# zhiqiangdon/pose-adv-aug

Measured on AMD Instinct MI355X. Metric: images/sec, 2-stack HG 256x256 bs=24 per GPU, full training step, higher is better.
Workload: dtype bf16; 1 GPU; BASELINE configs[1]: 2-stack hourglass chan 256, bs=24/GPU, 256x256 MPII-shape synthetic frames (720x1280 uint8 resident in HBM), on-device HumanAug warp, heat-map MSE, RMSprop, PCKh; global_batch=24, parallelism=dp1, ranks_seen=1, devices_seen=1

## Files before the change

### include/poseadv.h

```cpp
#ifndef POSEADV_H
#define POSEADV_H
#include <stddef.h>
#include <stdint.h>
#ifdef __cplusplus
extern "C" {
#endif

const char* pa_last_error(void);
int pa_version(void);
int pa_dtype(void);
float pa_grad_scale(void);


int pa_gaussian_heatmap(const double* pts, float* out, int B, int J, int H, int W, void* stream);

int pa_weighted_l2(const float* pred, const float* gt, const float* weight, size_t n, float* loss, void* stream);
int pa_weighted_l2_grad(const float* pred, const float* gt, const float* weight, size_t n, const float* gout_dev,
                        float* dpred, void* stream);

int pa_get_preds(const float* maps, int B, int J, int H, int W, float* preds, float* maxval, void* stream);

int pa_final_preds(const float* maps, const float* center, const float* scale, const float* rot,
                   int B, int J, int H, int W, float* out, float* scratch_preds, void* stream);

// ... 160 lines not shown
int pa_hg_set_dropout_masks(pa_net* net, const float* masks);

int pa_hg_accuracy(pa_net* net, int stack, const int32_t* idxs, int nidx, float* acc, float* scratch);

int pa_hg_pckh(pa_net* net, int stack, const float* center, const float* scale, const float* rot, const float* gt_pts,
               const float* norm, const int32_t* idxs, int nidx, float* acc, float* person, float* scratch);

int pa_net_meters_async(pa_net* net, int on);

#define PA_PROF_CLASSES 12
int pa_net_profile_begin(pa_net* net);
int pa_net_profile_report(pa_net* net, double* out_host, int cap_classes, int* n_classes);
int pa_net_profile_classes(const pa_net* net, int32_t* out_host, int cap);
int pa_net_set_fin_prologue(pa_net* net, int max_rows);
int pa_net_set_pool_route(pa_net* net, int on);
int pa_net_design_bytes(const pa_net* net, double* out_host);
int pa_copy_probe(void* dst, const void* src, size_t bytes, void* stream);
int pa_copy_probe_form(void* dst, const void* src, size_t bytes, int form, void* stream);
int pa_conv2d_time(int mode, int variant, int B, int Cin, int Cout, int H, int W, int k, int iters, void* ws, float* ms_out, void* stream);
int pa_conv_plan_describe(int B, int H, int W, int Cin, int Cout, int taps, int in_mode, int add1_mode, int add2_mode, int ep_mode,
                          int ep2_mode, int fin_rows, int flags, int cus, int* out, int cap);
int pa_conv_launch_log(int* out, int cap);

int pa_net_set_multi_stream(pa_net* net, int on);

int pa_hg_debug_tensor(pa_net* net, const char* which, int grad, float* out, int* shape4);

int pa_asn_debug_tensor(pa_net* net, const char* which, int grad, float* out, int* shape4);

#ifdef __cplusplus
// ... 4 lines not shown
```

### pose_adv_aug_amd/_lib.py

```python
import ctypes as C
import os

import torch

_HERE = os.path.dirname(os.path.abspath(__file__))
DTYPE = os.environ.get('POSEADV_DTYPE', 'bf16').lower()
if DTYPE not in ('bf16', 'fp16'):
    raise ValueError('POSEADV_DTYPE must be bf16 or fp16')
LIB_PATH = os.path.join(_HERE, 'libposeadv_hip.so' if DTYPE == 'bf16' else 'libposeadv_hip_fp16.so')


def set_dtype(name):
    global DTYPE, LIB_PATH
    name = name.lower()
    if name not in ('bf16', 'fp16'):
        raise ValueError('dtype must be bf16 or fp16')
    if _lib is not None and name != DTYPE:
        raise PoseAdvError('the %s library is already loaded in this process' % DTYPE)
    DTYPE = name
    LIB_PATH = os.path.join(_HERE, 'libposeadv_hip.so' if name == 'bf16' else 'libposeadv_hip_fp16.so')


def act_dtype():
    return torch.bfloat16 if DTYPE == 'bf16' else torch.float16
# ... 120 lines not shown
    'pa_hg_forward_half': (_i, [_vp, _vp, _vp, _i]),
    'pa_asn_forward': (_i, [_vp, _vp, _i, _vp, _vp]),
    'pa_asn_probs': (_vp, [_vp]),
    'pa_asn_backward': (_i, [_vp, _vp, _vp, _vp, _vp]),
    'pa_asn_set_log_eps': (_i, [_vp, _f]),
    'pa_hg_pckh': (_i, [_vp, _i, _vp, _vp, _vp, _vp, _vp, _vp, _i, _vp, _vp, _vp]),
    'pa_net_meters_async': (_i, [_vp, _i]),
    'pa_net_profile_begin': (_i, [_vp]),
    'pa_net_profile_report': (_i, [_vp, C.POINTER(C.c_double), _i, C.POINTER(_i)]),
    'pa_net_design_bytes': (_i, [_vp, C.POINTER(C.c_double)]),
    'pa_copy_probe': (_i, [_vp, _vp, _sz, _vp]),
    'pa_copy_probe_form': (_i, [_vp, _vp, _sz, _i, _vp]),
    'pa_params_csr': (_i, [_vp, _i, _vp, _vp]),
    'pa_net_set_fin_prologue': (_i, [_vp, _i]),
    'pa_net_set_pool_route': (_i, [_vp, _i]),
    'pa_wgrad_group_workspace_bytes': (_sz, [_vp, _i]),
    'pa_wgrad_group': (_i, [_vp, _i, _i, _vp, _vp]),
    'pa_conv2d_time': (_i, [_i] * 9 + [_vp, C.POINTER(C.c_float), _vp]),
    'pa_conv_plan_describe': (_i, [_i] * 14 + [C.POINTER(_i), _i]),
    'pa_conv_launch_log': (_i, [C.POINTER(_i), _i]),
    'pa_net_profile_classes': (_i, [_vp, C.POINTER(C.c_int32), _i]),
    'pa_net_set_multi_stream': (_i, [_vp, _i]),
    'pa_hg_debug_tensor': (_i, [_vp, C.c_char_p, _i, _vp, C.POINTER(_i)]),
    'pa_asn_debug_tensor': (_i, [_vp, C.c_char_p, _i, _vp, C.POINTER(_i)]),
}

EXPORTS = sorted(_PROTOS)


def lib():
# ... 49 lines not shown
```

### pose_adv_aug_amd/csrc/api.hip

```cpp
#include "../../include/poseadv.h"
#include "net.h"
#include "warp_bwd.h"
#include <stdio.h>
#include <string.h>
#include <new>
#include <string>

static thread_local char g_err[1024] = "";
void pa_set_error(const char* what, hipError_t e, const char* file, int line) {
    snprintf(g_err, sizeof g_err, "%s:%d: %s -> %s", file, line, what, hipGetErrorString(e));
}
void pa_set_error_msg(const char* msg) { snprintf(g_err, sizeof g_err, "%s", msg); }

struct pa_net { Net n; };
#define ST(s) reinterpret_cast<hipStream_t>(s)
#define TRY(x) do { int _r = (x); if (_r) { if (!g_err[0]) pa_set_error("kernel launch", (hipError_t)_r, __FILE__, __LINE__); return _r; } } while (0)

extern "C" {

const char* pa_last_error(void) { return g_err; }
float pa_grad_scale(void) { return PA_GRAD_SCALE; }
int pa_dtype(void) { return PA_DTYPE_ID; }
int pa_version(void) { return 1; }

// ... 810 lines not shown
    for (int c = 0; c < PA_PROF_NCLS && c < cap_classes; ++c)
        for (int j = 0; j < 4; ++j) out[c * 4 + j] = full[c * 4 + j];
    if (n_classes) *n_classes = PA_PROF_NCLS;
    return 0;
}
int pa_net_set_fin_prologue(pa_net* net, int max_rows) {
    net->n.fin_rows_max = max_rows < 0 ? 0 : (max_rows > PA_FIN_SMALL_ROWS ? PA_FIN_SMALL_ROWS : max_rows);
    net->n.release_graph();
    return 0;
}
int pa_net_set_pool_route(pa_net* net, int on) {
    net->n.pool_route = on ? 3 : 0;
    net->n.release_graph();
    return 0;
}
int pa_net_design_bytes(const pa_net* net, double* out) { out[0] = net->n.dbytes_rd; out[1] = net->n.dbytes_wr; return 0; }

int pa_net_profile_classes(const pa_net* net, int32_t* out, int cap) {
    const std::vector<int>& q = net->n.prof.last_seq;
    for (int i = 0; i < cap && i < (int)q.size(); ++i) out[i] = q[i];
    return (int)q.size();
}

int pa_net_set_multi_stream(pa_net* net, int on) {
    if (net->n.ensure_streams()) return 1;
    net->n.release_graph();
    net->n.multi_stream = on != 0 && net->n.side != nullptr;
    return 0;
}

// ... 64 lines not shown
                if (out && h.routed[k]) TRY(h.fill_poolgrad(n, k, n.xin[i]));
                head.raw = h.poolgrad[k]; head.B = x.B; head.H = x.H; head.W = x.W; head.C = x.C; a = &head;
            }
        } else {
            int k = r[r.find_first_of("1234")] - '1';
            std::string rest = r.substr(r.find_first_of("1234") + 1);
            if (r.rfind("skip", 0) == 0) a = pick_chain(h.skip[k], rest);
            else if (r.rfind("down", 0) == 0) a = pick_chain(h.down[k], rest);
            else if (r.rfind("up", 0) == 0) a = pick_chain(h.up[k], rest);
            else if (r.rfind("pool", 0) == 0) a = &h.pooled[k];
            else if (r.rfind("merge", 0) == 0) a = &h.merged[k];
        }
    }
    if (bad_block) { pa_set_error_msg("pa_hg_debug_tensor: no such block in the site's chain"); return 1; }
    if (!a) { pa_set_error_msg("pa_hg_debug_tensor: unknown tensor name"); return 1; }
    return debug_copy(n, *a, grad, out, shape4, "pa_hg_debug_tensor", mat);
}


int pa_asn_debug_tensor(pa_net* net, const char* which, int grad, float* out, int* shape4) {
    Net& n = net->n;
    std::string w(which);
    const Act* a = nullptr;
    const bf16* mat = nullptr;
    auto pick = [&](Residual& r, const std::string& rest) -> const Act* {
        if (rest == ".x1") return &r.x1;
        if (rest == ".x2") { mat = r.dz2_valid ? r.dz2 : nullptr; return &r.x2; }
        mat = r.dz3_valid ? r.dz3 : nullptr;
        return &r.x3;
    };
// ... 11 lines not shown
```

### pose_adv_aug_amd/csrc/conv_igemm.hip

```cpp
#include "common.h"
#include "kernels.h"
#include "common.h"
PA_STAMP_DECL(pa_conv1_clk, pa_debug_conv1_clocks)
#define PA_STAMP1(i) PA_STAMP_AT(pa_conv1_clk, a.dbg & 64, i)
#define PA_EPI_STAMP(i) PA_STAMP1(i)
#include "conv_epilogue.h"
#include <string.h>

template <int BM, int BN, int LDMODE, int TAPS, bool STEM = false, bool FIN = false>
__global__ __launch_bounds__(256, FIN ? 2 : 1) void conv_igemm_kernel(PaConvArgs a) {
    constexpr int AI = BM / 32, BI = BN / 32;
    constexpr int MI = BM / 32, NI = BN / 32;
    __shared__ __attribute__((aligned(16))) bf16 lds[(BM + BN) * 64];
    __shared__ float kst[LDMODE == PA_LD_PLAIN ? 4 : 3 * 512 + (FIN ? 2048 : 0)];
    bf16* As = lds;
    bf16* Bs = lds + BM * 64;
    const int tid = threadIdx.x, lane = tid & 63, wave = tid >> 6;
    const int wm = wave & 1, wn = wave >> 1;
    const int M = a.B * a.H * a.W, HW = a.H * a.W;
    const int K = TAPS * a.Cin;
    const int nK = K / 64;
    const int m0 = blockIdx.x * BM, n0 = blockIdx.y * BN;
    const int cc = tid & 7, r = tid >> 3;

// ... 281 lines not shown
}

template <int BM, int BN, int TAPS>
static void launch_ld(const PaConvArgs& a, int variant, dim3 grid, hipStream_t st) {
    if constexpr (BM == 64 && BN == 64) {
        if (variant == PA_CV_BNRELU_FIN) { hipLaunchKernelGGL((conv_igemm_kernel<BM, BN, PA_LD_BNRELU, TAPS, false, true>), grid, dim3(256), 0, st, a); return; }
        if (variant == PA_CV_LIN2_FIN) { hipLaunchKernelGGL((conv_igemm_kernel<BM, BN, PA_LD_LIN2, TAPS, false, true>), grid, dim3(256), 0, st, a); return; }
    }
    switch (variant) {
        case PA_LD_PLAIN: hipLaunchKernelGGL((conv_igemm_kernel<BM, BN, PA_LD_PLAIN, TAPS>), grid, dim3(256), 0, st, a); break;
        case PA_LD_BNRELU: hipLaunchKernelGGL((conv_igemm_kernel<BM, BN, PA_LD_BNRELU, TAPS>), grid, dim3(256), 0, st, a); break;
        default: hipLaunchKernelGGL((conv_igemm_kernel<BM, BN, PA_LD_LIN2, TAPS>), grid, dim3(256), 0, st, a); break;
    }
}

int pa_launch_stem_conv(const PaConvArgs& a, hipStream_t st, int* stat_rows) {
    if (a.Cin != 256 || a.Cout != 64 || a.in.mode != PA_LD_PLAIN) { pa_set_error_msg("pa_launch_stem_conv: bad arguments"); return 1; }
    const int M = a.B * a.H * a.W;
    const int bm = pa_conv_big_m(M) ? 128 : 64, rows = (M + bm - 1) / bm;
    if (stat_rows) *stat_rows = rows; if (a.ep.rows_out) *a.ep.rows_out = rows;
    if (bm == 128) hipLaunchKernelGGL((conv_igemm_kernel<128, 64, PA_LD_PLAIN, 1, true>), dim3(rows, 1), dim3(256), 0, st, a);
    else hipLaunchKernelGGL((conv_igemm_kernel<64, 64, PA_LD_PLAIN, 1, true>), dim3(rows, 1), dim3(256), 0, st, a);
    return (int)hipGetLastError();
}

static int g_log[1024][14], g_nlog = -1;
static void log_launch(const PaConvShape& s) {
    const int r[14] = {s.B, s.H, s.W, s.Cin, s.Cout, s.taps, s.in_mode, s.add1_mode, s.add2_mode, s.ep_mode, s.ep2_mode, s.fin_rows,
                       s.bias | s.out2 << 1 | s.want_dz << 2 | s.in_map << 3 | s.in_q << 4 | s.ep2_affine << 5 | s.add2_map << 6, s.cus};
    int i = 0; while (i < g_nlog && memcmp(g_log[i], r, sizeof r)) ++i;
    if (i == g_nlog && i < 1024) memcpy(g_log[g_nlog++], r, sizeof r);
}
int pa_launch_conv(const PaConvArgs& a0, const PaConvPlan& p, hipStream_t st, int* stat_rows) {
    if (p.path == PA_CVP_REFUSED) { pa_set_error_msg(p.why); return 1; }
    if (g_nlog >= 0) log_launch(pa_conv_shape(a0));
// ... 41 lines not shown
```

### pose_adv_aug_amd/csrc/kernels.h

```cpp
#pragma once
#include "common.h"
#include "bn_fin.h"
#include "launch_plan.h"
#include "wgrad_plan.h"
#include "conv_plan.h"

struct PaConvArgs {
    PaOperand in;
    const bf16* w;
    const float* bias;
    PaOperand add1;
    PaOperand add2;
    PaEpilogue ep;
    bf16* out;
    int B, H, W, Cin, Cout, taps;
    bf16* dz_out;
    PaBnFin fin;
    int low_prio;
    int dbg;
    int xcd;
    PaEpilogue ep2;
    bf16* out2;
};
int pa_conv_cus();
// ... 45 lines not shown
int pa_launch_bn_bwd_finalize(const float* bstats, int rows, const float* scale, const float* mean, const float* invstd,
                              float* kA, float* kB, float* kC, float* dgamma, float* dbeta, int C, float count,
                              hipStream_t st);

int pa_launch_maxpool_fwd(const PaOperand& in, bf16* out, int B, int H, int W, int C, hipStream_t st, unsigned char* map = nullptr, bf16* xmax = nullptr);
bool pa_pool_stats_route_supported(const PaOperand& in, const PaEpilogue& ep, int B, int H, int W, int C);
int pa_launch_maxpool_bwd_stats(const bf16* dout, const bf16* xmax, const PaOperand& in, const PaEpilogue& ep, int B, int H, int W, int C,
                                hipStream_t st, int* stat_rows = nullptr);
int pa_launch_maxpool_bwd(const bf16* dout, const PaOperand& in, const PaOperand& add, const PaEpilogue& ep, bf16* din,
                          int B, int H, int W, int C, hipStream_t st, int* stat_rows = nullptr);
int pa_launch_upadd_fwd(const PaOperand& low, const PaOperand& skip, bf16* out, int B, int H, int W, int C, hipStream_t st);
int pa_launch_upadd_bwd(const bf16* dout, const PaEpilogue& ep_low, bf16* dlow, const PaEpilogue& ep_skip, bf16* dskip,
                        int B, int H, int W, int C, hipStream_t st, int* stat_rows = nullptr, int part = 3);
bool pa_upadd_bwd_splits(const PaEpilogue& ep_low, const PaEpilogue& ep_skip, int B, int H, int W, int C);

int pa_launch_stem_conv(const PaConvArgs& a, hipStream_t st, int* stat_rows = nullptr);
int pa_launch_stem_wgrad(const PaWgradArgs& a, hipStream_t st);
int pa_launch_stem_wgrad_reduce(const float* part, int splits, float* dst, hipStream_t st, float* zero64 = nullptr);

struct PaStemDgradArgs {
    PaOperand g;
    const bf16* wf;
    float* out;
    int B, Hm, Wm, layout;
    float scale;
};
int pa_launch_stem_dgrad(const PaStemDgradArgs& a, hipStream_t st);
int pa_launch_stem_pack(const float* w, bf16* wf, hipStream_t st);

int pa_launch_rmsprop(float* p, const float* g, float* v, size_t n, float lr, float alpha, float eps, float gscale, int* state, hipStream_t st);
struct PaRmspropOpts { float lr, alpha, eps, mom, wd; };
// ... 26 lines not shown
```

### pose_adv_aug_amd/csrc/net.h

```cpp
#pragma once
#include <string>
#include <vector>
#include "common.h"
#include "kernels.h"
#include "pose_ops.h"

struct Arena {
    char* base = nullptr;
    size_t off = 0;
    void* take(size_t bytes) {
        off = (off + 255) & ~(size_t)255;
        void* p = base ? base + off : nullptr;
        off += bytes;
        return p;
    }
    template <typename T> T* get(size_t n) { return reinterpret_cast<T*>(take(n * sizeof(T))); }
};

struct TensorInfo {
    std::string name;
    int shape[4];
    int ndim;
    size_t offset;
    size_t numel;
// ... 8 lines not shown
    float *scale = nullptr, *shift = nullptr, *mean = nullptr, *invstd = nullptr;
    float *kA = nullptr, *kB = nullptr, *kC = nullptr;
    bool fin_pending = false, bfin_pending = false;
};

struct ConvLayer {
    int Cin = 0, Cout = 0, k = 1;
    int pcin = 0, pcout = 0;
    size_t p_w = 0, p_b = 0;
    bf16 *wf = nullptr, *wb = nullptr;
    float *part = nullptr, *dbpart = nullptr;
    int splits = 0;
    int red_index = -1;
    size_t part_floats = 0, db_floats = 0;
    bool has_bn_after = true;
    int taps() const { return k * k; }
};

struct Act {
    bf16* raw = nullptr;
    bf16* grad = nullptr;
    BNLayer* bn = nullptr;
    int B = 0, H = 0, W = 0, C = 0;
    size_t numel() const { return (size_t)B * H * W * C; }
    int M() const { return B * H * W; }
};

struct Net;

enum { PA_PROF_FWD1 = 0, PA_PROF_FWD3, PA_PROF_DGRAD1, PA_PROF_DGRAD3, PA_PROF_WGRAD1, PA_PROF_WGRAD3, PA_PROF_STEM_FWD,
// ... 170 lines not shown
    int finish_grad(const Act& a);
    int finish_grad2(const Act& a, const Act& b);
    int conv_fwd(ConvLayer& c, const PaOperand& in, int B, int H, int W, const PaOperand& add1, const PaOperand& add2,
                 bf16* out, BNLayer* bn_after, BNLayer* pending_in = nullptr, bool defer_after = false);
    int conv_dgrad(ConvLayer& c, const PaOperand& dy, int B, int H, int W, const PaOperand& add1, const PaOperand& add2,
                   const PaEpilogue& ep, bf16* out, bf16* dz_out = nullptr, bool* dz_done = nullptr, BNLayer* pending_in = nullptr,
                   const Act* low = nullptr, bool* low_done = nullptr,
                   const PaEpilogue* pool_in_ep = nullptr);
    int fin_rows_max = pa_tuning().fin_prologue > PA_FIN_SMALL_ROWS ? PA_FIN_SMALL_ROWS : pa_tuning().fin_prologue;
    int pool_route = pa_tuning().pool_route;
    bool maps_on = false;
    unsigned char* stem_map = nullptr; bf16* stem_xmax = nullptr;
    bool stem_map_written = false, stem_routed = false;
    bool stem_route_ok();
    int fill_stem_grad();
    int fin_mask = pa_tuning().fin_mask;
    bool fin_consumer_ok(const ConvLayer& c, int B, int H, int W, bool dgrad) const;
    PaBnFin fin_fwd(const BNLayer& b, int M) const;
    PaBnFin fin_bwd(const BNLayer& b, int M) const;
    int finish_grad_or_defer(const Act& a, bool defer);
    int finish_grad2_or_defer(const Act& a, bool defer_a, const Act& b, bool defer_b);
    bool x3_fin_ok(const Residual& r, const Act& in) const;
    bool x3_fin_ok(const Chain& c, const Act& in) const { return x3_fin_ok(c.tail(), c.tail_in(in)); }
    int conv_wgrad(ConvLayer& c, const PaOperand& dy, const PaOperand& x, int B, int H, int W);

    int prepare_weights();
    int begin_step();
    const bf16* cur_image = nullptr;
    int forward_pose(const float* img_nchw, const bf16* img4_in, const double* pts, bool train, float* loss_out_dev);
    int forward_pose_body(const float* img_nchw, const bf16* img4_in, const double* pts, bool train, float* loss_out_dev);
    int backward_pose();
    int backward_stack(int i);
    int backward_stem();
    hipEvent_t ev_bucket[16], ev_bucket_main = nullptr; bool bucket_events = false;
    int mark_bucket(int stack);
    int reduce_grads();
    int forward_half(const float* img_nchw, const bf16* img4_in, bool train);

    int scale_num = 7, rot_num = 7;
    Residual asn_in[5];
// ... 21 lines not shown
```

### pose_adv_aug_amd/csrc/net.hip

```cpp
#include "net.h"
#include <stdio.h>
#include <string.h>

static int ablate() { return pa_tuning().ablate; }
static int ablate_h() { return pa_tuning().ablate_h; }
#define TRY(x) do { int _r = (x); if (_r) return _r; } while (0)

PaOperand pa_plain(const bf16* p) { PaOperand o; o.p = p; o.q = nullptr; o.k0 = o.k1 = o.k2 = nullptr; o.map = nullptr; o.mode = PA_LD_PLAIN; return o; }
PaOperand pa_none() { PaOperand o; o.p = o.q = nullptr; o.k0 = o.k1 = o.k2 = nullptr; o.map = nullptr; o.mode = PA_LD_NONE; return o; }
static PaEpilogue ep_plain() { PaEpilogue e; memset(&e, 0, sizeof e); e.mode = PA_OUT_PLAIN; return e; }
static int round64(int v) { return (v + 63) / 64 * 64; }

size_t Net::add_param(const std::string& name, std::initializer_list<int> shape) {
    TensorInfo t; t.name = name; t.ndim = (int)shape.size(); t.is_buffer = 0;
    size_t n = 1; int i = 0;
    for (int s : shape) { t.shape[i++] = s; n *= (size_t)s; }
    for (; i < 4; ++i) t.shape[i] = 1;
    n_params = (n_params + 3) & ~(size_t)3;
    t.offset = n_params; t.numel = n;
    n_params += n;
    tensors.push_back(t);
    return t.offset;
}

// ... 185 lines not shown
        lgrad_tmp[i] = a.get<bf16>((size_t)M * chan);
        if (i + 1 < stacks) {
            layout_conv(forth[i], a, M, H4, H4); layout_conv(inc[i], a, M, H4, H4);
            forth_tmp[i] = a.get<bf16>((size_t)M * chan);
        }
        if (i == 0) xin[0] = res3.x3;
        if (i + 1 < stacks) xin[i + 1] = new_act(a, B, H4, H4, chan, nullptr, true);
    }
    a.take(0);
    return a.off;
}

int Net::upload_tables() {
    std::vector<PaPrepJob> pj; std::vector<PaWgradReduceJob> rj; std::vector<PaBnEvalJob> bj;
    prep_max = 0; red_max = 0;
    for (ConvLayer* c : convs) {
        PaPrepJob p; p.w = params + c->p_w; p.wf = c->wf; p.wb = c->wb; p.Cout = c->Cout; p.Cin = c->Cin;
        p.taps = c->k == 7 ? 49 : c->taps(); p.pad_cout = c->pcout; p.pad_cin = c->pcin;
        pj.push_back(p);
        int pe = c->pcout * (c->k == 7 ? 256 : c->taps() * c->pcin);
        if (pe > prep_max) prep_max = pe;
        if (c->k == 7) continue;
        PaWgradReduceJob r; r.part = c->part; r.dst = grads + c->p_w; r.dbpart = c->dbpart; r.dbdst = grads + c->p_b;
        r.Cout = c->pcout; r.Cin = c->pcin; r.taps = c->taps(); r.splits = c->splits; r.real_cout = c->Cout; r.real_cin = c->Cin;
        c->red_index = (int)rj.size();
        rj.push_back(r);
        int re = c->Cout * c->Cin * c->taps() + c->Cout;
        if (re > red_max) red_max = re;
    }
    for (BNLayer* b : bns) {
// ... 120 lines not shown
    f.scale = b.scale; f.shift = b.shift; f.mean = b.mean; f.invstd = b.invstd;
    f.momentum = momentum; f.eps = eps; f.update_running = bn_update;
    return f;
}

PaBnFin Net::fin_bwd(const BNLayer& b, int M) const {
    PaBnFin f; memset(&f, 0, sizeof f);
    f.stats = b.bstats; f.rows = b.bstat_rows; f.bwd = 1; f.count = (float)M;
    f.scale = b.scale; f.mean = b.mean; f.invstd = b.invstd;
    f.kA = b.kA; f.kB = b.kB; f.kC = b.kC; f.dgamma = grads + b.p_gamma; f.dbeta = grads + b.p_beta;
    return f;
}

int Net::conv_fwd(ConvLayer& c, const PaOperand& in, int B_, int H, int W, const PaOperand& add1, const PaOperand& add2,
                  bf16* out, BNLayer* bn_after, BNLayer* pending_in, bool defer_after) {
    PaConvArgs a; memset(&a, 0, sizeof a);
    if (pending_in && pending_in->fin_pending) { a.fin = fin_fwd(*pending_in, B_ * H * W); pending_in->fin_pending = false; }
    a.in = in; a.w = c.wf; a.bias = params + c.p_b; a.add1 = add1; a.add2 = add2; a.out = out; a.low_prio = on_side ? 1 : 0;
    a.B = B_; a.H = H; a.W = W; a.Cin = c.pcin; a.Cout = c.pcout; a.taps = c.k == 7 ? 1 : c.taps();
    a.ep = ep_plain();
    if (bn_after && train_bn) { a.ep.mode = PA_OUT_STATS; a.ep.stats = bn_after->stats; a.ep.rows_out = &bn_after->stat_rows; }
    double wb, wf; conv_work(B_ * H * W, c.k == 7 ? 147 : c.Cin, c.Cout, c.k == 7 ? 1 : c.taps(), false, wb, wf);
    if (c.k == 7) wb = 2.0 * B_ * (4.0 * H * W * 4 + (double)H * W * 64) + 2.0 * 64 * 147;
    if ((ablate() & 128) && H <= ablate_h()) return 0;
    { const double M = (double)B_ * H * W;
      cnt((c.k == 7 ? 2.0 * B_ * 4.0 * H * W * 4 : opb(in, M * a.Cin)) + opb(add1, M * a.Cout) + opb(add2, M * a.Cout) + 2.0 * a.Cout * a.taps * a.Cin, 2.0 * M * a.Cout); }
    ProfEntry* pe = prof.begin(c.k == 7 ? PA_PROF_STEM_FWD : ((long)B_ * H * W < PA_PROF_LOW_M ? PA_PROF_LOW_FWD : (c.k == 3 ? PA_PROF_FWD3 : PA_PROF_FWD1)), wb, wf, st);
    int rc = (c.k == 3 && (ablate() & 8)) ? 0 : ((c.k == 7) ? pa_launch_stem_conv(a, st) : pa_launch_conv(a, st));
    prof.end(pe, st);
    TRY(rc);
    if (bn_after && train_bn && defer_after && bn_after->stat_rows > 0 && bn_after->stat_rows <= fin_rows_max) { bn_after->fin_pending = true; return 0; }
    if (bn_after && train_bn && !(ablate() & 4))
        TRY(pa_launch_bn_finalize(bn_after->stats, bn_after->stat_rows, params + bn_after->p_gamma, params + bn_after->p_beta,
                                  buffers + bn_after->b_rmean, buffers + bn_after->b_rvar, bn_after->scale, bn_after->shift,
                                  bn_after->mean, bn_after->invstd, bn_after->C, (float)(B_ * H * W), momentum, eps, bn_update, st));
    return 0;
}

int Net::conv_dgrad(ConvLayer& c, const PaOperand& dy, int B_, int H, int W, const PaOperand& add1, const PaOperand& add2,
                    const PaEpilogue& ep, bf16* out, bf16* dz_out, bool* dz_done, BNLayer* pending_in, const Act* low, bool* low_done,
                    const PaEpilogue* pool_in_ep) {
    PaConvArgs a; memset(&a, 0, sizeof a);
    if (low_done) *low_done = false;
    if (pending_in && pending_in->bfin_pending) { a.fin = fin_bwd(*pending_in, B_ * H * W); pending_in->bfin_pending = false; }
    a.in = dy; a.w = c.wb; a.bias = nullptr; a.add1 = add1; a.add2 = add2; a.out = out; a.ep = ep; a.low_prio = on_side ? 1 : 0;
    a.B = B_; a.H = H; a.W = W; a.Cin = c.pcout; a.Cout = c.pcin; a.taps = c.taps();
    if (dy.mode == PA_LD_POOL) {
        if (!pool_in_ep || !dz_out) { pa_set_error_msg("conv_dgrad: a pool-routed gradient needs its mask and a dz buffer"); return 1; }
        a.ep2 = *pool_in_ep;
    }
    if (dy.mode == PA_LD_POOL || dy.mode == PA_LD_LIN2) a.dz_out = dz_out;
    if (low && dy.mode != PA_LD_POOL && pa_tuning().upadd_fuse && low->bn && !drop_mask && !(ablate() & 1024)) { a.out2 = low->grad; a.ep2 = final_ep(*low); }
    PaConvPlan p = pa_conv_plan(pa_conv_shape(a));
    if (a.out2 && p.path != PA_CVP_ROW_UP) { a.out2 = nullptr; memset(&a.ep2, 0, sizeof a.ep2); p = pa_conv_plan(pa_conv_shape(a)); }
    const bool up = p.path == PA_CVP_ROW_UP; if (dz_done) *dz_done = p.stores_dz;
    double wb, wf; conv_work(B_ * H * W, c.Cin, c.Cout, c.taps(), false, wb, wf);
// ... 383 lines not shown
        }
        if (k >= 1) TRY(n.finish_grad_or_defer(x, n.x3_fin_ok(down[k - 1], pooled[k - 1])));
        else TRY(n.finish_grad(x));
    }
    return 0;
}

int Net::ensure_streams() {
    if (streams_ready) return 0;
    if (pa_tuning().single_stream) { streams_ready = true; return 0; }
    PA_CHECK(hipStreamCreateWithFlags(&side, hipStreamNonBlocking));
    for (int k = 0; k < 4; ++k) {
        PA_CHECK(hipEventCreateWithFlags(&ev_fork[k], hipEventDisableTiming));
        PA_CHECK(hipEventCreateWithFlags(&ev_join[k], hipEventDisableTiming));
    }
    if (!pa_tuning().no_wstream) {
        PA_CHECK(hipStreamCreateWithFlags(&wstream, hipStreamNonBlocking));
        for (int i = 0; i < 16; ++i) PA_CHECK(hipEventCreateWithFlags(&ev_w[i], hipEventDisableTiming));
        PA_CHECK(hipEventCreateWithFlags(&ev_wdone, hipEventDisableTiming));
    }
    streams_ready = true;
    return 0;
}
void Net::release_streams() {
    release_graph();
    if (bucket_events) { for (int i = 0; i < 16; ++i) (void)hipEventDestroy(ev_bucket[i]); (void)hipEventDestroy(ev_bucket_main); bucket_events = false; }
    if (mstream) { (void)hipStreamSynchronize(mstream); (void)hipStreamDestroy(mstream); (void)hipEventDestroy(ev_mfork); (void)hipEventDestroy(ev_meter); mstream = nullptr; meter_pending = false; }
    if (side) {
        (void)hipStreamSynchronize(side); (void)hipStreamDestroy(side); side = nullptr;
        for (int k = 0; k < 4; ++k) { (void)hipEventDestroy(ev_fork[k]); (void)hipEventDestroy(ev_join[k]); }
    }
    if (wstream) {
        (void)hipStreamSynchronize(wstream); (void)hipStreamDestroy(wstream); wstream = nullptr;
        for (int i = 0; i < 16; ++i) (void)hipEventDestroy(ev_w[i]);
        (void)hipEventDestroy(ev_wdone);
    }
    for (ProfEntry& e : prof.entries) { (void)hipEventDestroy(e.e0); (void)hipEventDestroy(e.e1); }
    prof.entries.clear(); prof.used = 0;
    streams_ready = false;
}
int Net::fork_to(int k) { PA_CHECK(hipEventRecord(ev_fork[k], st)); PA_CHECK(hipStreamWaitEvent(side, ev_fork[k], 0)); return 0; }
int Net::record_join(int k) { PA_CHECK(hipEventRecord(ev_join[k], side)); return 0; }
int Net::wait_join(int k) { PA_CHECK(hipStreamWaitEvent(st, ev_join[k], 0)); return 0; }

int Net::prepare_weights() { return pa_launch_weight_prep(prep_jobs, n_prep, prep_max, st); }

int Net::begin_step() {
    dbytes_rd = dbytes_wr = 0;
    if (!loss_self_clearing) PA_CHECK(hipMemsetAsync(stats_arena, 0, stats_arena_floats * sizeof(float), st));
    return 0;
}

int Net::meter_stream(hipStream_t* out) {
    *out = st;
    if (!meters_async || !multi_stream) return join_meters();
    if (!mstream) {
        PA_CHECK(hipStreamCreateWithFlags(&mstream, hipStreamNonBlocking));
        PA_CHECK(hipEventCreateWithFlags(&ev_mfork, hipEventDisableTiming));
        PA_CHECK(hipEventCreateWithFlags(&ev_meter, hipEventDisableTiming));
    }
// ... 43 lines not shown
    if (!img4_in) TRY(pa_launch_nchw_to_nhwc4(img_nchw, img4, B, res, res, st));
    if (pts && pts != pts_dev) PA_CHECK(hipMemcpyAsync(pts_dev, pts, (size_t)B * classes * 2 * sizeof(double), hipMemcpyDeviceToDevice, st));
    TRY(conv_fwd(stem_conv, pa_plain(image), B, res / 2, res / 2, pa_none(), pa_none(), a0.raw, &stem_bn));
    TRY(res1.fwd(*this, a0));
    maps_on = (pool_route & 1) && train;
    stem_map_written = (pool_route & 2) && train && stem_map && pa_pool_stats_route_supported(op(res1.x3), final_ep(res1.x3), B, res / 2, res / 2, 128);
    TRY(c_maxpool_fwd(*this, op(res1.x3), pool0.raw, B, res / 2, res / 2, 128, st, stem_map_written ? stem_map : nullptr, stem_map_written ? stem_xmax : nullptr));
    TRY(res2.fwd(*this, pool0));
    TRY(res3.fwd(*this, res2.x3));
    const int Hh = res / 4;
    for (int i = 0; i < stacks; ++i) {
        TRY(hg[i].encode(*this, xin[i]));
        TRY(hg[i].decode(*this));
        TRY(post[i].fwd(*this, hg[i].out()));
        TRY(conv_fwd(lin[i], op(post[i].out()), B, Hh, Hh, pa_none(), pa_none(), lin_out[i].raw, &lin_bn[i]));
        TRY(c_head_fwd(*this, op(lin_out[i]), outc[i].wf, params + outc[i].p_b, heat[i], heat64[i], pts ? pts_dev : nullptr,
                               pts ? loss_dev + i : nullptr, B, Hh, Hh, chan, st));
        if (i + 1 < stacks) {
            TRY(conv_fwd(forth[i], op(lin_out[i]), B, Hh, Hh, op(xin[i]), pa_none(), forth_tmp[i], nullptr));
            TRY(conv_fwd(inc[i], pa_plain(heat64[i]), B, Hh, Hh, pa_plain(forth_tmp[i]), pa_none(), xin[i + 1].raw, nullptr));
        }
    }
    if (pts) TRY(pa_launch_loss_out(loss_dev, loss_keep, loss_out_dev, loss_total_out, stacks, st));
    return 0;
}

int Net::backward_stack(int i) {
    const int Hh = res / 4;
    const float gscale = PA_GRAD_SCALE / ((float)B * 16.f * (float)Hh * (float)Hh);
    const bool inner = i + 1 < stacks;
// ... 20 lines not shown
    TRY(finish_grad(lin_out[i]));
    PaOperand gl = gradop(lin_out[i]);
    bool gl_stored = false;
    TRY(conv_dgrad(lin[i], gl, B, Hh, Hh, pa_none(), pa_none(), final_ep(post[i].out()), post[i].out().grad, lgrad_tmp[i], &gl_stored));
    if (gl_stored) gl = pa_plain(lgrad_tmp[i]);
    TRY(conv_wgrad(lin[i], gl, op(post[i].out()), B, Hh, Hh));
    TRY(finish_grad(post[i].out()));
    post[i].head().low_of_in = hg[i].low_fusable(*this, 0) ? &hg[i].up[0].out() : nullptr;
    TRY(post[i].bwd(*this, hg[i].out(), pa_none(), true));
    hg[i].low_done[0] = post[i].head().low_fused;
    TRY(hg[i].bwd(*this, xin[i], inner ? pa_plain(xin[i + 1].grad) : pa_none()));
    return 0;
}

int Net::backward_stem() {
    TRY(res3.bwd(*this, res2.x3, pa_none(), true));
    TRY(finish_grad(res2.x3));
    TRY(res2.bwd(*this, pool0, pa_none(), true));
    stem_routed = stem_route_ok();
    res1.g3_pool_on = stem_routed;
    if (stem_routed) {
        const double e = (double)B * (res / 4) * (res / 4) * 128;
        cnt(4.0 * e, 0.0);
        TRY(pa_launch_maxpool_bwd_stats(pool0.grad, stem_xmax, op(res1.x3), final_ep(res1.x3), B, res / 2, res / 2, 128, st));
        TRY(finish_grad(res1.x3));
        res1.g3_pool = gradop(res1.x3);
        res1.g3_pool.mode = PA_LD_POOL; res1.g3_pool.p = pool0.grad; res1.g3_pool.map = stem_map;
        res1.g3_pool_ep = final_ep(res1.x3);
    } else {
        TRY(c_maxpool_bwd(*this, pool0.grad, op(res1.x3), pa_none(), final_ep(res1.x3), res1.x3.grad, B, res / 2, res / 2, 128, st));
// ... 45 lines not shown
    }
    TRY(flush_wgrads());
    if (!wgrads_aside()) return -1;
    TRY(flush_red_stash(wstream));
    PA_CHECK(hipEventRecord(ev_bucket_main, st));
    PA_CHECK(hipStreamWaitEvent(wstream, ev_bucket_main, 0));
    PA_CHECK(hipEventRecord(ev_bucket[stack], wstream));
    return 0;
}

int Net::train_step_graph(bool train) {
    TRY(ensure_streams());
    const int key = (train ? 1 : 0) | (multi_stream ? 2 : 0);
    if (drop_mask || prof.on) { pa_set_error_msg("train_step_graph: not with the occlusion branch / the launch profiler"); return 1; }
    TRY(join_meters());
    if (!step_exec || step_key != key) {
        release_graph();
        hipStream_t cap = nullptr, caller = st;
        PA_CHECK(hipStreamCreateWithFlags(&cap, hipStreamNonBlocking));
        st = cap;
        hipError_t e = hipStreamBeginCapture(cap, hipStreamCaptureModeRelaxed);
        capturing = e == hipSuccess;
        if (e != hipSuccess) { st = caller; (void)hipStreamDestroy(cap); pa_set_error("hipStreamBeginCapture", e, __FILE__, __LINE__); return (int)e; }
        int rc = forward_pose(nullptr, img4, pts_dev, train, nullptr);
        if (!rc) rc = backward_pose();
        hipGraph_t g = nullptr;
        e = hipStreamEndCapture(cap, &g);
        capturing = false;
        st = caller;
        (void)hipStreamDestroy(cap);
// ... 34 lines not shown
```

### pose_adv_aug_amd/csrc/tuning.h

```cpp
#pragma once
#include <stdlib.h>

#define PA_TUNING_TABLE(X)                                                                                                           \
                                                                      \
    X(conv1_old,        "PA_CONV1_OLD",        0,   "1x1 convolutions on the generic kernel (no row-tile kernel, no fused upsample-add gradient)") \
    X(conv3_old,        "PA_CONV3_OLD",        0,   "3x3 convolutions on the generic kernel (no halo-tile kernel)")                 \
    X(wgrad_old,        "PA_WGRAD_OLD",        0,   "weight gradients on the generic kernel (no tile kernel, stem included)")       \
    X(stem_wgrad_old,   "PA_STEM_WGRAD_OLD",   0,   "the stem's weight gradient on the generic kernel")                            \
    X(eltwise_old,      "PA_ELTWISE_OLD",      0,   "pooling / upsample-add / cell-mask launches in their first, unvectorised form") \
    X(conv3_nosmall,    "PA_CONV3_NOSMALL",    0,   "no 8 x 8 / 4 x 4 halo tiles: the small maps go to the generic kernel")        \
    X(igemm_oneshot,    "PA_IGEMM_ONESHOT",    1,   "0: the small 1x1 layers on the K-stepping generic kernel instead of the one-shot one") \
    X(no_dz3,           "PA_NO_DZ3",           0,   "conv3's data gradient does not store dz3 (its readers recompute it)")         \
    X(no_dz2,           "PA_NO_DZ2",           0,   "conv2's data gradient does not store dz2")                                    \
    X(epi_bwd_direct,   "PA_EPI_BWD_DIRECT",   0,   "direct (no LDS) BatchNorm-backward epilogue wherever an instance carries both") \
    X(conv3_noxcd,      "PA_CONV3_NOXCD",      0,   "3x3 tiles in launch order instead of one contiguous range per XCD")           \
    X(wg_group,         "PA_WG_GROUP",         1,   "0: one launch per weight gradient instead of group launches")                 \
    X(wg_red_in_group,  "PA_WG_RED_IN_GROUP",  1,   "0: slab reductions as launches of their own instead of inside the next group launch") \
    X(wgrad_anyorder,   "PA_WGRAD_ANYORDER",   1,   "0: ungrouped weight gradients of one flush as ordinary in-order launches")    \
    X(wgrad_nopipe,     "PA_WGRAD_NOPIPE",     0,   "plain instead of pipelined tile weight gradients")                            \
    X(upadd_fuse,       "PA_UPADD_FUSE",       1,   "0: the upsample-add backward's low-resolution half as a launch of its own")   \
    X(upadd_split,      "PA_UPADD_SPLIT",      1,   "0: both halves of the upsample-add backward in one launch on the main stream") \
    X(pool_route,       "PA_POOL_ROUTE",       3,   "pool gradients through the forward pools' arg-max maps: bit 0 the hourglass pools, bit 1 the stem's pool (0: a pool backward launch each)") \
    X(fin_prologue,     "PA_FIN_PROLOGUE",     128, "most partial rows a consumer finalizes in its prologue (0: always a finalize launch; at most 128)") \
    X(fin_mask,         "PA_FIN_MASK",         7,   "which finalizes may ride in a consumer: 1 forward x1 / x2, 2 backward x2, 4 backward x3") \
    X(single_stream,    "PA_SINGLE_STREAM",    0,   "everything on the caller's stream")                                           \
    X(no_wstream,       "PA_NO_WSTREAM",       0,   "side streams, but the weight gradients on the stream that produced their operands") \
    X(stem_on_main,     "PA_STEM_ON_MAIN",     1,   "0: the stem's weight gradient on the weight-gradient stream")                 \
                                                              \
    X(wgrad_wgs1,       "PA_WGRAD_WGS1",       256, "workgroup target of a 1x1 tile weight gradient launched alone")               \
    X(wgrad_wgs9,       "PA_WGRAD_WGS9",       256, "the same for 3x3")                                                            \
    X(wgrad_min1,       "PA_WGRAD_MIN1",       3,   "fewest 128-pixel tiles for which a 1x1 weight gradient takes the tile kernel") \
    X(wg_group_wgs1,    "PA_WG_GROUP_WGS1",    64,  "workgroup budget of a 1x1 job of a group launch")                             \
    X(wg_group_wgs9,    "PA_WG_GROUP_WGS9",    64,  "the same for 3x3")                                                            \
    X(wg_group_minper1, "PA_WG_GROUP_MINPER1", 2,   "fewest tiles per workgroup of a 1x1 job")                                     \
    X(wg_group_minper9, "PA_WG_GROUP_MINPER9", 4,   "the same for 3x3")                                                            \
    X(wg_group_cap,     "PA_WG_GROUP_CAP",     256, "most workgroups of one group launch")                                         \
    X(wg_red_wgs,       "PA_WG_RED_WGS",       256, "workgroups of the slab reduction inside a group launch")                      \
    X(wreduce_lag,      "PA_WREDUCE_LAG",      2,   "flushes whose slabs wait in the stash before they are summed")                \
    X(stem_splits,      "PA_STEM_SPLITS",      512, "splits (slabs) of the stem's weight gradient")                                \
    X(wgrad_tile1,      "PA_WGRAD_TILE1",      0,   "generic 1x1 weight gradient: forced tile variant (0: by shape)")              \
    X(wgrad_tile9,      "PA_WGRAD_TILE9",      0,   "the same for 3x3")                                                            \
    X(wgrad_blocks,     "PA_WGRAD_BLOCKS",     0,   "generic weight gradient: forced split count (0: by shape)")                   \
// ... 32 lines not shown
```

Baseline: 4251 images/sec.

## Add dedicated stem forward kernel and overlap weight re-pack with forward

Adds a specialised 7x7 stride-2 stem forward kernel that gathers input patches into registers and stages K through LDS in quarters (or halves) before MFMA. It also splits the per-step weight re-pack: the first five convs' weights are repacked on the main stream and the rest on the side stream, with each later conv waiting on an event before it uses its weights. The intent is to shorten the stem launch and hide the weight-prep launch behind the early forward layers. The cost is extra event synchronisation and more code paths. The overlap is skipped during graph capture or graph replay.

After: 4266 images/sec, median of 6. No clear change (+0.4%).

```diff
diff --git a/include/poseadv.h b/include/poseadv.h
--- a/include/poseadv.h
+++ b/include/poseadv.h
@@ -198,6 +198,9 @@
 int pa_net_profile_classes(const pa_net* net, int32_t* out_host, int cap);
 int pa_net_set_fin_prologue(pa_net* net, int max_rows);
 int pa_net_set_pool_route(pa_net* net, int on);
+int pa_net_set_stem_kernel(pa_net* net, int on);
+int pa_net_set_prep_overlap(pa_net* net, int on);
+int pa_net_debug_weight_copies(pa_net* net, void* out, size_t cap_bytes, size_t* bytes);
 int pa_net_design_bytes(const pa_net* net, double* out_host);
 int pa_copy_probe(void* dst, const void* src, size_t bytes, void* stream);
 int pa_copy_probe_form(void* dst, const void* src, size_t bytes, int form, void* stream);
diff --git a/pose_adv_aug_amd/_lib.py b/pose_adv_aug_amd/_lib.py
--- a/pose_adv_aug_amd/_lib.py
+++ b/pose_adv_aug_amd/_lib.py
@@ -158,6 +158,9 @@
     'pa_params_csr': (_i, [_vp, _i, _vp, _vp]),
     'pa_net_set_fin_prologue': (_i, [_vp, _i]),
     'pa_net_set_pool_route': (_i, [_vp, _i]),
+    'pa_net_set_stem_kernel': (_i, [_vp, _i]),
+    'pa_net_set_prep_overlap': (_i, [_vp, _i]),
+    'pa_net_debug_weight_copies': (_i, [_vp, _vp, _sz, C.POINTER(_sz)]),
     'pa_wgrad_group_workspace_bytes': (_sz, [_vp, _i]),
     'pa_wgrad_group': (_i, [_vp, _i, _i, _vp, _vp]),
     'pa_conv2d_time': (_i, [_i] * 9 + [_vp, C.POINTER(C.c_float), _vp]),
diff --git a/pose_adv_aug_amd/csrc/api.hip b/pose_adv_aug_amd/csrc/api.hip
--- a/pose_adv_aug_amd/csrc/api.hip
+++ b/pose_adv_aug_amd/csrc/api.hip
@@ -848,6 +848,28 @@
     net->n.release_graph();
     return 0;
 }
+int pa_net_set_stem_kernel(pa_net* net, int on) {
+    net->n.stem_kernel = on;
+    net->n.release_graph();
+    return 0;
+}
+int pa_net_set_prep_overlap(pa_net* net, int on) { net->n.prep_overlap = on != 0; return 0; }
+int pa_net_debug_weight_copies(pa_net* net, void* out, size_t cap_bytes, size_t* bytes) {
+    Net& n = net->n;
+    size_t total = 0;
+    for (const ConvLayer* c : n.convs) total += (size_t)c->pcout * (c->k == 7 ? 256 : c->taps() * c->pcin) * sizeof(bf16) * (c->wb ? 2 : 1);
+    if (bytes) *bytes = total;
+    if (!out) return 0;
+    if (cap_bytes < total) { pa_set_error_msg("pa_net_debug_weight_copies: out is too small"); return 1; }
+    TRY(n.join_prep());
+    char* o = static_cast<char*>(out);
+    for (const ConvLayer* c : n.convs) {
+        const size_t b = (size_t)c->pcout * (c->k == 7 ? 256 : c->taps() * c->pcin) * sizeof(bf16);
+        PA_CHECK(hipMemcpyAsync(o, c->wf, b, hipMemcpyDeviceToDevice, n.st)); o += b;
+        if (c->wb) { PA_CHECK(hipMemcpyAsync(o, c->wb, b, hipMemcpyDeviceToDevice, n.st)); o += b; }
+    }
+    return 0;
+}
 int pa_net_design_bytes(const pa_net* net, double* out) { out[0] = net->n.dbytes_rd; out[1] = net->n.dbytes_wr; return 0; }
 
 int pa_net_profile_classes(const pa_net* net, int32_t* out, int cap) {
@@ -942,6 +964,14 @@
     }
     if (bad_block) { pa_set_error_msg("pa_hg_debug_tensor: no such block in the site's chain"); return 1; }
     if (!a) { pa_set_error_msg("pa_hg_debug_tensor: unknown tensor name"); return 1; }
+    if (grad == 5) {
+        if (!a->bn) { pa_set_error_msg("pa_hg_debug_tensor: this tensor has no pending BatchNorm"); return 1; }
+        const BNLayer& b = *a->bn;
+        shape4[0] = 4; shape4[1] = b.C; shape4[2] = shape4[3] = 1;
+        const float* src[4] = {b.scale, b.shift, b.mean, b.invstd};
+        for (int i = 0; out && i < 4; ++i) PA_CHECK(hipMemcpyAsync(out + (size_t)i * b.C, src[i], sizeof(float) * b.C, hipMemcpyDeviceToDevice, n.st));
+        return 0;
+    }
     return debug_copy(n, *a, grad, out, shape4, "pa_hg_debug_tensor", mat);
 }
 
diff --git a/pose_adv_aug_amd/csrc/conv_igemm.hip b/pose_adv_aug_amd/csrc/conv_igemm.hip
--- a/pose_adv_aug_amd/csrc/conv_igemm.hip
+++ b/pose_adv_aug_amd/csrc/conv_igemm.hip
@@ -319,11 +319,12 @@
     }
 }
 
-int pa_launch_stem_conv(const PaConvArgs& a, hipStream_t st, int* stat_rows) {
+int pa_launch_stem_conv(const PaConvArgs& a, hipStream_t st, int* stat_rows, int kernel) {
     if (a.Cin != 256 || a.Cout != 64 || a.in.mode != PA_LD_PLAIN) { pa_set_error_msg("pa_launch_stem_conv: bad arguments"); return 1; }
     const int M = a.B * a.H * a.W;
     const int bm = pa_conv_big_m(M) ? 128 : 64, rows = (M + bm - 1) / bm;
     if (stat_rows) *stat_rows = rows; if (a.ep.rows_out) *a.ep.rows_out = rows;
+    if (bm == 128 && kernel) return pa_launch_stem_fwd(a, rows, kernel == 2 ? 2 : 4, st);
     if (bm == 128) hipLaunchKernelGGL((conv_igemm_kernel<128, 64, PA_LD_PLAIN, 1, true>), dim3(rows, 1), dim3(256), 0, st, a);
     else hipLaunchKernelGGL((conv_igemm_kernel<64, 64, PA_LD_PLAIN, 1, true>), dim3(rows, 1), dim3(256), 0, st, a);
     return (int)hipGetLastError();
diff --git a/pose_adv_aug_amd/csrc/kernels.h b/pose_adv_aug_amd/csrc/kernels.h
--- a/pose_adv_aug_amd/csrc/kernels.h
+++ b/pose_adv_aug_amd/csrc/kernels.h
@@ -83,7 +83,8 @@
                         int B, int H, int W, int C, hipStream_t st, int* stat_rows = nullptr, int part = 3);
 bool pa_upadd_bwd_splits(const PaEpilogue& ep_low, const PaEpilogue& ep_skip, int B, int H, int W, int C);
 
-int pa_launch_stem_conv(const PaConvArgs& a, hipStream_t st, int* stat_rows = nullptr);
+int pa_launch_stem_conv(const PaConvArgs& a, hipStream_t st, int* stat_rows = nullptr, int kernel = 1);
+int pa_launch_stem_fwd(const PaConvArgs& a, int rows, int nh, hipStream_t st);
 int pa_launch_stem_wgrad(const PaWgradArgs& a, hipStream_t st);
 int pa_launch_stem_wgrad_reduce(const float* part, int splits, float* dst, hipStream_t st, float* zero64 = nullptr);
 
diff --git a/pose_adv_aug_amd/csrc/net.h b/pose_adv_aug_amd/csrc/net.h
--- a/pose_adv_aug_amd/csrc/net.h
+++ b/pose_adv_aug_amd/csrc/net.h
@@ -46,6 +46,7 @@
     int red_index = -1;
     size_t part_floats = 0, db_floats = 0;
     bool has_bn_after = true;
+    bool prep_head = false;
     int taps() const { return k * k; }
 };
 
@@ -246,6 +247,7 @@
     bool stem_map_written = false, stem_routed = false;
     bool stem_route_ok();
     int fill_stem_grad();
+    int stem_kernel = pa_tuning().stem_kernel;
     int fin_mask = pa_tuning().fin_mask;
     bool fin_consumer_ok(const ConvLayer& c, int B, int H, int W, bool dgrad) const;
     PaBnFin fin_fwd(const BNLayer& b, int M) const;
@@ -256,6 +258,12 @@
     bool x3_fin_ok(const Chain& c, const Act& in) const { return x3_fin_ok(c.tail(), c.tail_in(in)); }
     int conv_wgrad(ConvLayer& c, const PaOperand& dy, const PaOperand& x, int B, int H, int W);
 
+    int prep_overlap = pa_tuning().prep_overlap, n_prep_head = 0;
+    hipEvent_t ev_prep_fork = nullptr, ev_prep_done = nullptr;
+    bool prep_pending = false;
+    bool bwd_since_prep = false;
+    int join_prep();
+    int need_weights(const ConvLayer& c) { return prep_pending && !c.prep_head ? join_prep() : 0; }
     int prepare_weights();
     int begin_step();
     const bf16* cur_image = nullptr;
diff --git a/pose_adv_aug_amd/csrc/net.hip b/pose_adv_aug_amd/csrc/net.hip
--- a/pose_adv_aug_amd/csrc/net.hip
+++ b/pose_adv_aug_amd/csrc/net.hip
@@ -223,6 +223,12 @@
 int Net::upload_tables() {
     std::vector<PaPrepJob> pj; std::vector<PaWgradReduceJob> rj; std::vector<PaBnEvalJob> bj;
     prep_max = 0; red_max = 0;
+    n_prep_head = 0;
+    if (!is_agent) {
+        for (ConvLayer* c : {&stem_conv, &res1.c1, &res1.c2, &res1.c3, &res1.ad}) c->prep_head = true;
+        while (n_prep_head < (int)convs.size() && convs[n_prep_head]->prep_head) ++n_prep_head;
+        if (n_prep_head != 5) n_prep_head = 0;
+    }
     for (ConvLayer* c : convs) {
         PaPrepJob p; p.w = params + c->p_w; p.wf = c->wf; p.wb = c->wb; p.Cout = c->Cout; p.Cin = c->Cin;
         p.taps = c->k == 7 ? 49 : c->taps(); p.pad_cout = c->pcout; p.pad_cin = c->pcin;
@@ -373,6 +379,7 @@
 
 int Net::conv_fwd(ConvLayer& c, const PaOperand& in, int B_, int H, int W, const PaOperand& add1, const PaOperand& add2,
                   bf16* out, BNLayer* bn_after, BNLayer* pending_in, bool defer_after) {
+    TRY(need_weights(c));
     PaConvArgs a; memset(&a, 0, sizeof a);
     if (pending_in && pending_in->fin_pending) { a.fin = fin_fwd(*pending_in, B_ * H * W); pending_in->fin_pending = false; }
     a.in = in; a.w = c.wf; a.bias = params + c.p_b; a.add1 = add1; a.add2 = add2; a.out = out; a.low_prio = on_side ? 1 : 0;
@@ -385,7 +392,7 @@
     { const double M = (double)B_ * H * W;
       cnt((c.k == 7 ? 2.0 * B_ * 4.0 * H * W * 4 : opb(in, M * a.Cin)) + opb(add1, M * a.Cout) + opb(add2, M * a.Cout) + 2.0 * a.Cout * a.taps * a.Cin, 2.0 * M * a.Cout); }
     ProfEntry* pe = prof.begin(c.k == 7 ? PA_PROF_STEM_FWD : ((long)B_ * H * W < PA_PROF_LOW_M ? PA_PROF_LOW_FWD : (c.k == 3 ? PA_PROF_FWD3 : PA_PROF_FWD1)), wb, wf, st);
-    int rc = (c.k == 3 && (ablate() & 8)) ? 0 : ((c.k == 7) ? pa_launch_stem_conv(a, st) : pa_launch_conv(a, st));
+    int rc = (c.k == 3 && (ablate() & 8)) ? 0 : ((c.k == 7) ? pa_launch_stem_conv(a, st, nullptr, stem_kernel) : pa_launch_conv(a, st));
     prof.end(pe, st);
     TRY(rc);
     if (bn_after && train_bn && defer_after && bn_after->stat_rows > 0 && bn_after->stat_rows <= fin_rows_max) { bn_after->fin_pending = true; return 0; }
@@ -399,6 +406,7 @@
 int Net::conv_dgrad(ConvLayer& c, const PaOperand& dy, int B_, int H, int W, const PaOperand& add1, const PaOperand& add2,
                     const PaEpilogue& ep, bf16* out, bf16* dz_out, bool* dz_done, BNLayer* pending_in, const Act* low, bool* low_done,
                     const PaEpilogue* pool_in_ep) {
+    TRY(need_weights(c));
     PaConvArgs a; memset(&a, 0, sizeof a);
     if (low_done) *low_done = false;
     if (pending_in && pending_in->bfin_pending) { a.fin = fin_bwd(*pending_in, B_ * H * W); pending_in->bfin_pending = false; }
@@ -812,6 +820,8 @@
         PA_CHECK(hipEventCreateWithFlags(&ev_fork[k], hipEventDisableTiming));
         PA_CHECK(hipEventCreateWithFlags(&ev_join[k], hipEventDisableTiming));
     }
+    PA_CHECK(hipEventCreateWithFlags(&ev_prep_fork, hipEventDisableTiming));
+    PA_CHECK(hipEventCreateWithFlags(&ev_prep_done, hipEventDisableTiming));
     if (!pa_tuning().no_wstream) {
         PA_CHECK(hipStreamCreateWithFlags(&wstream, hipStreamNonBlocking));
         for (int i = 0; i < 16; ++i) PA_CHECK(hipEventCreateWithFlags(&ev_w[i], hipEventDisableTiming));
@@ -827,6 +837,7 @@
     if (side) {
         (void)hipStreamSynchronize(side); (void)hipStreamDestroy(side); side = nullptr;
         for (int k = 0; k < 4; ++k) { (void)hipEventDestroy(ev_fork[k]); (void)hipEventDestroy(ev_join[k]); }
+        (void)hipEventDestroy(ev_prep_fork); (void)hipEventDestroy(ev_prep_done); ev_prep_fork = ev_prep_done = nullptr; prep_pending = false;
     }
     if (wstream) {
         (void)hipStreamSynchronize(wstream); (void)hipStreamDestroy(wstream); wstream = nullptr;
@@ -841,7 +852,27 @@
 int Net::record_join(int k) { PA_CHECK(hipEventRecord(ev_join[k], side)); return 0; }
 int Net::wait_join(int k) { PA_CHECK(hipStreamWaitEvent(st, ev_join[k], 0)); return 0; }
 
-int Net::prepare_weights() { return pa_launch_weight_prep(prep_jobs, n_prep, prep_max, st); }
+int Net::join_prep() {
+    if (!prep_pending || (on_side && st == side)) return 0;
+    PA_CHECK(hipStreamWaitEvent(st, ev_prep_done, 0));
+    prep_pending = false;
+    return 0;
+}
+
+int Net::prepare_weights() {
+    TRY(join_prep());
+    const bool overlap = prep_overlap && bwd_since_prep && multi_stream && side && ev_prep_done && !capturing && !step_exec &&
+                         n_prep_head > 0 && n_prep_head < n_prep;
+    bwd_since_prep = false;
+    if (!overlap) return pa_launch_weight_prep(prep_jobs, n_prep, prep_max, st);
+    PA_CHECK(hipEventRecord(ev_prep_fork, st));
+    TRY(pa_launch_weight_prep(prep_jobs, n_prep_head, prep_max, st));
+    PA_CHECK(hipStreamWaitEvent(side, ev_prep_fork, 0));
+    TRY(pa_launch_weight_prep(prep_jobs + n_prep_head, n_prep - n_prep_head, prep_max, side));
+    PA_CHECK(hipEventRecord(ev_prep_done, side));
+    prep_pending = true;
+    return 0;
+}
 
 int Net::begin_step() {
     dbytes_rd = dbytes_wr = 0;
@@ -915,6 +946,7 @@
         TRY(hg[i].decode(*this));
         TRY(post[i].fwd(*this, hg[i].out()));
         TRY(conv_fwd(lin[i], op(post[i].out()), B, Hh, Hh, pa_none(), pa_none(), lin_out[i].raw, &lin_bn[i]));
+        TRY(need_weights(outc[i]));
         TRY(c_head_fwd(*this, op(lin_out[i]), outc[i].wf, params + outc[i].p_b, heat[i], heat64[i], pts ? pts_dev : nullptr,
                                pts ? loss_dev + i : nullptr, B, Hh, Hh, chan, st));
         if (i + 1 < stacks) {
@@ -965,6 +997,7 @@
 }
 
 int Net::backward_stem() {
+    bwd_since_prep = true;
     TRY(res3.bwd(*this, res2.x3, pa_none(), true));
     TRY(finish_grad(res2.x3));
     TRY(res2.bwd(*this, pool0, pa_none(), true));
@@ -1040,6 +1073,7 @@
     const int key = (train ? 1 : 0) | (multi_stream ? 2 : 0);
     if (drop_mask || prof.on) { pa_set_error_msg("train_step_graph: not with the occlusion branch / the launch profiler"); return 1; }
     TRY(join_meters());
+    TRY(join_prep());
     if (!step_exec || step_key != key) {
         release_graph();
         hipStream_t cap = nullptr, caller = st;
diff --git a/pose_adv_aug_amd/csrc/stem_fwd.hip b/pose_adv_aug_amd/csrc/stem_fwd.hip
--- /dev/null
+++ b/pose_adv_aug_amd/csrc/stem_fwd.hip
@@ -0,0 +1,104 @@
+#include "common.h"
+#include "kernels.h"
+#include "conv_epilogue.h"
+
+template <int NH>
+__global__ __launch_bounds__(256, NH == 4 ? 3 : 2) void stem_fwd_kernel(PaConvArgs a) {
+    constexpr int BM = 128, BN = 64, MI = 4, NI = 2;
+    constexpr int KT = 4 / NH;
+    constexpr int JP = 16 / NH;
+    __shared__ __attribute__((aligned(16))) bf16 lds[BN * 256 + KT * BM * 64];
+    bf16* Bs = lds;
+    bf16* As = lds + BN * 256;
+    const int tid = threadIdx.x, lane = tid & 63, wave = tid >> 6;
+    const int wm = wave & 1, wn = wave >> 1;
+    const int M = a.B * a.H * a.W, HW = a.H * a.W;
+    const int m0 = blockIdx.x * BM;
+    const int Hin = 2 * a.H, Win = 2 * a.W;
+
+    bf16x8 rw[8];
+    const int wc = tid & 31, wr = tid >> 5;
+#pragma unroll
+    for (int i = 0; i < 8; ++i) rw[i] = *reinterpret_cast<const bf16x8*>(a.w + (size_t)(wr + 8 * i) * 256 + wc * 8);
+
+    const int p = tid & 127, h = tid >> 7;
+    const bool ok = m0 + p < M;
+    const int m = ok ? m0 + p : 0;
+    const int pb = m / HW, rem = m - pb * HW, py = rem / a.W, px = rem - py * a.W;
+    bf16x4 lo[14], hi[14];
+    unsigned lmask = 0, hmask = 0;
+#pragma unroll
+    for (int j = 0; j < 14; ++j) {
+        const int ky = j >> 1, q = 2 * (j & 1) + h;
+        const int yi = 2 * py + ky - 3, xi = 2 * px + 2 * q - 3;
+        const bool rowok = ok && (unsigned)yi < (unsigned)Hin;
+        const bool lok = rowok && (unsigned)xi < (unsigned)Win, hok = rowok && (unsigned)(xi + 1) < (unsigned)Win;
+        const bf16* rowp = a.in.p + ((size_t)pb * Hin + (rowok ? yi : 0)) * Win * 4;
+        lo[j] = *reinterpret_cast<const bf16x4*>(rowp + (size_t)(lok ? xi : 0) * 4);
+        hi[j] = *reinterpret_cast<const bf16x4*>(rowp + (size_t)(hok ? xi + 1 : 0) * 4);
+        lmask |= (lok ? 1u : 0u) << j; hmask |= (hok ? 1u : 0u) << j;
+    }
+
+#pragma unroll
+    for (int i = 0; i < 8; ++i) {
+        const int lrow = pa_lds_row_of_weight_row<BN, NI>(wr + 8 * i);
+        *reinterpret_cast<bf16x8*>(Bs + (wc >> 3) * (BN * 64) + lrow * 64 + (((wc & 7) ^ (lrow & 7)) << 3)) = rw[i];
+    }
+
+    f32x4 acc[NI][MI];
+#pragma unroll
+    for (int ni = 0; ni < NI; ++ni)
+#pragma unroll
+        for (int mi = 0; mi < MI; ++mi) acc[ni][mi] = f32x4{0.f, 0.f, 0.f, 0.f};
+    const int frow = lane & 15, fchk = lane >> 4;
+    const bf16x4 z4 = {(bf16)0.f, (bf16)0.f, (bf16)0.f, (bf16)0.f};
+
+#pragma unroll
+    for (int ph = 0; ph < NH; ++ph) {
+        if (ph) __syncthreads();
+#pragma unroll
+        for (int jj = 0; jj < JP; ++jj) {
+            const int j = ph * JP + jj;
+            bf16x8 o = __builtin_shufflevector(z4, z4, 0, 1, 2, 3, 4, 5, 6, 7);
+            if (j < 14) {
+                const int js = j < 14 ? j : 0;
+                const bf16x4 l = (lmask >> js) & 1 ? lo[js] : z4, u = (hmask >> js) & 1 ? hi[js] : z4;
+                o = __builtin_shufflevector(l, u, 0, 1, 2, 3, 4, 5, 6, 7);
+            }
+            const int cidx = 2 * j + h;
+            *reinterpret_cast<bf16x8*>(As + ((cidx >> 3) - ph * KT) * (BM * 64) + p * 64 + (((cidx & 7) ^ (p & 7)) << 3)) = o;
+        }
+        __syncthreads();
+#pragma unroll
+        for (int kt = 0; kt < KT; ++kt)
+#pragma unroll
+            for (int kk = 0; kk < 2; ++kk) {
+                bf16x8 fa[MI], fw[NI];
+#pragma unroll
+                for (int mi = 0; mi < MI; ++mi) {
+                    const int row = wm * (BM / 2) + mi * 16 + frow;
+                    fa[mi] = *reinterpret_cast<const bf16x8*>(As + kt * (BM * 64) + row * 64 + (((fchk + 4 * kk) ^ (row & 7)) << 3));
+                }
+#pragma unroll
+                for (int ni = 0; ni < NI; ++ni) {
+                    const int row = wn * (BN / 2) + ni * 16 + frow;
+                    fw[ni] = *reinterpret_cast<const bf16x8*>(Bs + (ph * KT + kt) * (BN * 64) + row * 64 + (((fchk + 4 * kk) ^ (row & 7)) << 3));
+                }
+#pragma unroll
+                for (int ni = 0; ni < NI; ++ni)
+#pragma unroll
+                    for (int mi = 0; mi < MI; ++mi)
+                        acc[ni][mi] = PA_MFMA_16x16x32(fw[ni], fa[mi], acc[ni][mi]);
+            }
+    }
+    __syncthreads();
+    pa_conv_epilogue_auto<BN, NI, MI>(a, acc, 0, wm, wn,
+                                     [&](int wr_, int mi, int q) { const int mm = m0 + wr_ * (BM / 2) + mi * 16 + q; return mm < M ? mm : -1; },
+                                     reinterpret_cast<float*>(lds), (int)blockIdx.x);
+}
+
+int pa_launch_stem_fwd(const PaConvArgs& a, int rows, int nh, hipStream_t st) {
+    if (nh == 2) hipLaunchKernelGGL((stem_fwd_kernel<2>), dim3(rows, 1), dim3(256), 0, st, a);
+    else hipLaunchKernelGGL((stem_fwd_kernel<4>), dim3(rows, 1), dim3(256), 0, st, a);
+    return (int)hipGetLastError();
+}
diff --git a/pose_adv_aug_amd/csrc/tuning.h b/pose_adv_aug_amd/csrc/tuning.h
--- a/pose_adv_aug_amd/csrc/tuning.h
+++ b/pose_adv_aug_amd/csrc/tuning.h
@@ -26,6 +26,8 @@
     X(single_stream,    "PA_SINGLE_STREAM",    0,   "everything on the caller's stream")                                           \
     X(no_wstream,       "PA_NO_WSTREAM",       0,   "side streams, but the weight gradients on the stream that produced their operands") \
     X(stem_on_main,     "PA_STEM_ON_MAIN",     1,   "0: the stem's weight gradient on the weight-gradient stream")                 \
+    X(stem_kernel,      "PA_STEM_KERNEL",      1,   "0: the stem's forward on the generic kernel instead of stem_fwd.hip; 2: stem_fwd.hip with K staged in halves")         \
+    X(prep_overlap,     "PA_PREP_OVERLAP",     1,   "0: the weight re-pack of a training step as one launch on the main stream")   \
                                                               \
     X(wgrad_wgs1,       "PA_WGRAD_WGS1",       256, "workgroup target of a 1x1 tile weight gradient launched alone")               \
     X(wgrad_wgs9,       "PA_WGRAD_WGS9",       256, "the same for 3x3")                                                            \
```
